# pingooio/pingoo

Measured on AMD Instinct MI355X. Metric: requests/sec matched (whole node), 1k-rule WAF, higher is better.
Workload: dtype u8

## Files before the change

pingoo_amd/build.py:

```python
from __future__ import annotations

import os
import shutil
import subprocess
import sys

HERE = os.path.dirname(os.path.abspath(__file__))
CSRC = os.path.join(HERE, "csrc")
LIB = os.path.join(HERE, "libpwaf.so")
SOURCES = ["frontend.cpp", "pattern.cpp", "dfa.cpp", "iptrie.cpp", "filter.cpp", "residual.cpp", "residual_jit.cpp", "rtc.cpp", "compile.cpp", "loaders.cpp", "batcher.cpp", "async.cpp", "node.cpp", "engine.cpp", "kernels.hip", "records.hip"]
HEADERS = ["frontend.h", "program.h", "kernels.h", "residual.h", "confirm.h", "records.h", "lscan_split.h", "unicode_data.inc", os.path.join("..", "..", "include", "pwaf.h")]


def hipcc() -> str:
    for cand in (os.environ.get("HIPCC"), shutil.which("hipcc"), "/opt/rocm/bin/hipcc"):
        if cand and os.path.exists(cand):
            return cand
    raise RuntimeError("hipcc not found (needed to build pingoo_amd/libpwaf.so)")


EMBED = os.path.join(CSRC, "residual_h.inc")


def embed() -> str:
    text = open(os.path.join(CSRC, "residual.h")).read()
    assert ')RVMH"' not in text
    out = 'R"RVMH(' + text + ')RVMH"\n'
    if not os.path.exists(EMBED) or open(EMBED).read() != out:
        with open(EMBED, "w") as f:
            f.write(out)
    return EMBED


def is_stale(lib: str = LIB) -> bool:
    if not os.path.exists(lib):
        return True
    t = os.path.getmtime(lib)
    return any(os.path.getmtime(os.path.join(CSRC, f)) > t for f in SOURCES + HEADERS)


def build(force: bool = False, verbose: bool = False, variant: str = "") -> str:
    lib = LIB if not variant else os.path.join(HERE, f"libpwaf_{variant}.so")
    if not force and not is_stale(lib):
        return lib
# ... 40 lines not shown
```

pingoo_amd/csrc/engine.cpp:

```cpp
#include <hip/hip_runtime_api.h>

#include <cstdio>
#include <algorithm>
#include <cstring>
#include <functional>
#include <map>
#include <memory>
#include <mutex>
#include <string>
#include <unordered_map>
#include <vector>

#include "frontend.h"
#include "kernels.h"
#include "lscan_split.h"
#include "program.h"
#include "records.h"

using namespace pwaf;

struct pwaf_program {
    std::unique_ptr<Program> p;
    std::vector<uint8_t> dump;
};
// ... 1227 lines not shown
                la[phase].push_back(a);
            }
            if (d.confirm && !d.confirm_walk) continue;
#ifdef PWAF_PROFILING
            if (skip_identity_walks() && d.identity) continue;
#endif
            ListScanArgs a = list_args(gi, lshapes[phase]);
            if (phase == 0 && d.confirm && dense_flag_of[gi] != nullptr) {
                a.dense_flag = dense_flag_of[gi];
                a.dense_thresh = dense_thresh_of[gi];
                a.dense_mode = 2;
            } else if (d.share_owner >= 0 && dense_flag_of[(size_t)d.share_owner] != nullptr) {
                a.dense_flag = dense_flag_of[(size_t)d.share_owner];
                a.dense_thresh = dense_thresh_of[(size_t)d.share_owner];
                a.dense_mode = 3;
            }
            la[phase].push_back(a);
        }
    for (int phase = 0; phase < 2; phase++) {
        size_t planned = 0;
        for (const uint32_t c : e->lscan_launches[phase]) planned += c;
        if (planned != la[phase].size()) return fail(PWAF_E_DEVICE, "list-scan launch plan does not match the batch's descriptors");
    }
    ColPtrChunk ptrs{};
    if (P.n_residual) {
        const size_t nc = e->n_fields;
        ptrs.count = (uint32_t)(2 * nc);
        for (size_t f = 0; f < nc; f++) { ptrs.p[f] = cols[f].data; ptrs.p[nc + f] = cols[f].offsets; }
    }
    const uint32_t nf = (uint32_t)fall.size(), nc_conf = (uint32_t)call.size();
    const FilterArgs *d_all = nullptr, *d_s1 = nullptr, *d_s2 = nullptr;
    const ConfirmArgs *d_c = nullptr;
    const ListScanArgs *d_la[2] = {nullptr, nullptr};
    uint32_t *c_plan = nullptr, *l_plan = nullptr;
    {
        size_t ab = 0;
        auto part = [&](size_t bytes) { const size_t at = ab; ab = (ab + bytes + 255) & ~(size_t)255; return at; };
        const size_t a_all = part((size_t)nf * sizeof(FilterArgs)), a_s1 = part(by_stride[0].size() * sizeof(FilterArgs)), a_s2 = part(by_stride[1].size() * sizeof(FilterArgs)),
                     a_c = part((size_t)nc_conf * sizeof(ConfirmArgs)), a_l0 = part((la[0].size() + 1) * sizeof(ListScanArgs)), a_l1 = part((la[1].size() + 1) * sizeof(ListScanArgs)),
                     a_ptrs = part((size_t)ptrs.count * sizeof(void *));
        const size_t up_bytes = ab;
        const size_t a_cplan = part(((size_t)nc_conf + 2) * 4), a_lplan = part((lsplit::plan_words(e->lscan_launches[0]) + lsplit::plan_words(e->lscan_launches[1])) * 4);
        if ((rc = S.args.reserve(ab))) return rc;
        char *const abase = (char *)S.args.p;
        d_all = (const FilterArgs *)(abase + a_all);
        d_s1 = (const FilterArgs *)(abase + a_s1);
        d_s2 = (const FilterArgs *)(abase + a_s2);
        d_c = (const ConfirmArgs *)(abase + a_c);
        d_la[0] = (const ListScanArgs *)(abase + a_l0);
        d_la[1] = (const ListScanArgs *)(abase + a_l1);
        S.res_cols.p = abase + a_ptrs;
        c_plan = (uint32_t *)(abase + a_cplan);
        l_plan = (uint32_t *)(abase + a_lplan);
        if (up_bytes) {
            const uint32_t slot = S.arg_next++ % Scratch::kArgSlots;
            if (S.arg_pending[slot]) HIP_TRY(hipEventSynchronize(S.arg_ev[slot]));
            if ((rc = S.arg_slot[slot].reserve(up_bytes))) return rc;
            char *const hb = (char *)S.arg_slot[slot].p;
            auto put = [&](size_t at, const void *src, size_t bytes) { if (bytes) memcpy(hb + at, src, bytes); };
            put(a_all, fall.data(), (size_t)nf * sizeof(FilterArgs));
            put(a_s1, by_stride[0].data(), by_stride[0].size() * sizeof(FilterArgs));
            put(a_s2, by_stride[1].data(), by_stride[1].size() * sizeof(FilterArgs));
            put(a_c, call.data(), (size_t)nc_conf * sizeof(ConfirmArgs));
            put(a_l0, la[0].data(), la[0].size() * sizeof(ListScanArgs));
            put(a_l1, la[1].data(), la[1].size() * sizeof(ListScanArgs));
            put(a_ptrs, ptrs.p, (size_t)ptrs.count * sizeof(void *));
            int he = upload_args_block(hb, S.args.p, up_bytes, zero_deferred ? S.zero_block.p : nullptr, zero_deferred ? zero_bytes : 0, stream);
            if (he) return fail(PWAF_E_DEVICE, std::string("descriptor upload failed: ") + hipGetErrorString((hipError_t)he));
            zero_deferred = false;
            arg_slot_used = (int)slot;
        }
        if (zero_deferred) {
            HIP_TRY(hipMemsetAsync(S.zero_block.p, 0, zero_bytes, stream));
            zero_deferred = false;
        }
    }
    if (e->n_filtered) {
        int he;
        stream_mark = true;
        if ((rc = mark(nullptr, 0))) return rc;
        he = launch_filter(by_stride[0].data(), (uint32_t)by_stride[0].size(), d_s1, by_stride[1].data(), (uint32_t)by_stride[1].size(), d_s2, stream);
        if (he) return fail(PWAF_E_DEVICE, std::string("filter kernel launch failed: ") + hipGetErrorString((hipError_t)he));
        if ((rc = mark(by_stride[1].empty() ? "filter_s1" : by_stride[0].empty() ? "filter_s2" : "filter_mix", alg_bytes[1] + alg_bytes[2]))) return rc;
        stream_mark = false;
#ifdef PWAF_PROFILING
        static const bool attr_after_compact = getenv("PWAF_ATTR_AFTER_COMPACT") != nullptr;
        if (!attr_after_compact)
#endif
        if ((rc = launch_attr_side())) return rc;
        if ((rc = mark(nullptr, 0))) return rc;
        he = launch_resolve(fall.data(), nf, d_all, stream);
        bool any_list = false;
        for (const DevGroup &d : e->groups) any_list = any_list || (d.filtered && !d.confirm);
        if (!he && any_list) he = launch_compact(fall.data(), nf, d_all, stream);
        if (he) return fail(PWAF_E_DEVICE, std::string("resolve / compact kernel launch failed: ") + hipGetErrorString((hipError_t)he));
        if ((rc = mark("resolve+compact", 0xFCu))) return rc;
        if (!call.empty()) {
            if ((rc = mark(nullptr, 0))) return rc;
            he = launch_confirm(call.data(), nc_conf, d_c, c_plan, e->n_cus, stream);
            if (he) return fail(PWAF_E_DEVICE, std::string("confirm kernel launch failed: ") + hipGetErrorString((hipError_t)he));
            if ((rc = mark("confirm", 0xF8u))) return rc;
        }
    }
    if ((rc = launch_attr_side())) return rc;
    {
        uint32_t *plan_at = l_plan;
        for (int phase = 0; phase < 2; phase++) {
            uint32_t first = 0;
            for (const uint32_t cnt : e->lscan_launches[phase]) {
                if ((rc = mark(nullptr, 0))) return rc;
                int he = launch_scan_gated(la[phase].data() + first, cnt, d_la[phase] + first, plan_at, lshapes[phase], stream);
                plan_at += 2 * cnt + 1;
                first += cnt;
                if (he) return fail(PWAF_E_DEVICE, std::string("gated scan kernel launch failed: ") + hipGetErrorString((hipError_t)he));
                char nm[48];
                snprintf(nm, sizeof nm, "lscan_x%u", cnt);
                if ((rc = mark(nm, 0xFDu))) return rc;
            }
        }
    }
    if (!P.fcmp.empty()) {
        FcmpArgs fa{};
        std::vector<uint32_t> slots;
        for (size_t k = 0; k < P.fcmp.size(); k++) {
            uint32_t sl[2];
            const uint32_t fld[2] = {P.fcmp[k].a, P.fcmp[k].b};
            for (int q = 0; q < 2; q++) {
                size_t at = std::find(slots.begin(), slots.end(), fld[q]) - slots.begin();
                if (at == slots.size()) slots.push_back(fld[q]);
                sl[q] = (uint32_t)at;
            }
            fa.atoms[k] = P.fcmp[k].op | (sl[0] << 8) | (sl[1] << 16);
        }
        for (size_t q = 0; q < slots.size() && q < kMaxFcmpFields; q++) {
            fa.data[q] = cols[slots[q]].data;
            fa.off[q] = cols[slots[q]].offsets;
        }
        fa.n = n;
        fa.n_atoms = (uint32_t)P.fcmp.size();
        fa.rec = (uint32_t *)S.rec.p + e->groups.size() * (size_t)n;
        fa.pool = (PoolEntry *)S.pool.p;
        fa.pool_count = (uint32_t *)S.ctrl.p;
        fa.pool_cap = pool_cap;
        fa.status = status_word;
        if ((rc = mark(nullptr, 0))) return rc;
// ... 1466 lines not shown
```

pingoo_amd/csrc/kernels.h:

```cpp
#pragma once
#include <cstdint>
#include <string>
#include <vector>

#include "program.h"

namespace pwaf {

static constexpr int kMaxPasses = 250;
static constexpr int kVerdictPre = 12;
static constexpr uint32_t kGapLists = 32;
static constexpr uint32_t kMaxHeaderLens = 8;
static constexpr uint32_t kDirChunkWords = 32;

static constexpr uint32_t REC_OVERFLOW = 0x80000000u;
struct PoolEntry {
    uint32_t atom;
    uint32_t next;
};

struct SpecialCell {
    uint32_t next_off;
    uint32_t emit;
};
// ... 83 lines not shown
    uint32_t pair_cap;
    uint32_t mul, stride, init;
    const uint32_t *ftable;
    const uint32_t *c_head;
    const ConfirmEntry *c_entries;
    const uint8_t *c_bytes;
    const uint32_t *c_classes;
    uint32_t n_entries, n_bytes, n_class_words;
    uint32_t *rec;
    uint32_t *valid_bits;
    uint32_t *walk_bits;
    uint32_t *walk_list;
    uint32_t *walk_count;
    PoolEntry *pool;
    uint32_t *pool_count;
    uint32_t pool_cap;
    uint32_t *status;
    const uint32_t *colmask_local;
    uint32_t n_local;
    uint32_t *gate_lists;
    uint32_t *gate_count;
    uint32_t *enq_bits;
    uint32_t enq_words;
    uint32_t shared_bits;
    const uint32_t *dense_flag;
    uint32_t dense_thresh;
};
static constexpr uint32_t kConfirmThreads = 1024;
static constexpr uint32_t kConfirmPoolBytes = 40 * 1024;
struct ConfirmTableDev {
    const ConfirmArgs *c;
    uint32_t count;
};
int launch_confirm(const ConfirmArgs *host, uint32_t count, const ConfirmArgs *dev, uint32_t *plan, uint32_t n_cus, void *stream);

static constexpr uint32_t kStreamSlab = 128 * 1024;
static constexpr uint32_t kStreamIter = 4096;
static constexpr uint32_t kFilterWaves = 4;
static constexpr uint32_t kCompactWords = 2048;
struct FilterArgs {
    const uint8_t *data;
    const uint32_t *off;
    uint32_t n;
    uint32_t total;
    uint32_t slab0;
    uint32_t init;
    uint32_t mul;
    uint32_t stride;
    const uint32_t *table;
    uint32_t n_heads;
    uint32_t head_w[2][4];
    uint32_t head_m[2][4];
    uint32_t head_len[2];
    uint32_t head_code[2];
    uint32_t *rec;
    uint32_t *chunk_bits;
    uint32_t *sub_count;
    uint32_t *bitmap;
    uint32_t *block_count;
    uint32_t *list;
    uint32_t *list_count;
    uint2 *pairs;
    uint32_t *pair_count;
    uint32_t pair_cap;
    uint32_t *pair_base;
    const uint32_t *dense_flag;
    uint32_t dense_thresh;
// ... 147 lines not shown
    const uint32_t *dir24;
    const uint32_t *dir_chunks, *dir_vals;
    const uint32_t *dir_summary;
    uint32_t dir_sum_shift, dir_common;
    const uint2 *dir_esc;
    const uint32_t *class_rows;
    uint32_t class_words;
    uint32_t acmp_words;
    uint32_t geo_default;
    uint32_t *ipres;
    uint32_t ipres_packed;
    uint32_t has_geo;
    uint4 *gpairs;
    uint32_t *ghdr;
    uint32_t pair_stride;
    uint32_t attr_blocks;
    pwaf_verdict *out;
    unsigned long long *counts;
    uint32_t *match_idx;
    uint32_t *n_matches;
};

int launch_scan(const ScanArgs &a, void *stream);
struct GatedTable {
    const ListScanArgs *g;
    uint32_t count;
    uint32_t debug;
};
struct ListShape {
    uint32_t threads, hot_bytes, wg_per_cu;
};
ListShape list_shape(uint32_t variant);
uint32_t list_hot_bytes(const ListShape &shape);
int launch_scan_gated(const ListScanArgs *host, uint32_t count, const ListScanArgs *dev, uint32_t *plan, const ListShape &shape, void *stream);
int launch_verdict(const VerdictArgs &a, void *stream);
int launch_ipres(const VerdictArgs &a, void *stream);
int launch_attr(const VerdictArgs &a, void *stream);
int launch_dir24(const VerdictArgs &a, void *out , void *esc, void *esc_count, void *stream);
uint32_t scan_lds_bytes(uint32_t n_hot, uint32_t stride, uint32_t n_gate_atoms);
struct VerdictShape {
    uint32_t waves, lds_bytes, lds_tables;
    uint32_t sparse, v_cap, per_cu;
};
VerdictShape verdict_shape(uint32_t n_cols, uint32_t n_rules, uint32_t n_trig, uint32_t n_lits, bool force_global = false, int mode = 3, uint32_t n_passes = 0);
uint32_t verdict_blocks_sp(const VerdictShape &sh, uint32_t n_cus);

}
```

pingoo_amd/csrc/kernels.hip:

```cpp
#include <hip/hip_runtime.h>

#include <cstdlib>
#include <mutex>
#include <set>

#include "confirm.h"
#include "utf8.h"
#include "kernels.h"
#include "residual.h"

namespace pwaf {

static constexpr int kScanThreads = 1024;
static constexpr int kScanWaves = kScanThreads / 64;
static constexpr uint32_t kNone = 0xFFFFFFFFu;

#define PWAF_LDS __attribute__((address_space(3)))
#define PWAF_GLOBAL __attribute__((address_space(1)))
typedef const PWAF_LDS uint16_t *lds_u16_ptr;
typedef const PWAF_GLOBAL uint16_t *glb_u16_ptr;
typedef const PWAF_LDS uint32_t *lds_u32_ptr;
typedef const PWAF_LDS uint8_t *lds_u8_ptr;
typedef unsigned int u32x4 __attribute__((ext_vector_type(4)));
typedef u32x4 u32x4_u __attribute__((aligned(1)));

static constexpr uint32_t kClsBytes = 1024;
uint32_t scan_lds_bytes(uint32_t n_hot, uint32_t stride, uint32_t n_gate_atoms) {
    const uint32_t need = (((n_hot + 1) * stride * 2 + 15) & ~15u) + kClsBytes + n_gate_atoms * 4;
    const uint32_t reach = ((0xFFFFu << 1) + stride * 2 + kClsBytes + 15) & ~15u;
    return need > reach ? need : reach;
}


struct Hits {
    uint32_t a0, a1;
    uint32_t ovf;
};

struct SlowCtx {
    const uint32_t *list_off;
    const uint16_t *list;
    PoolEntry *pool;
// ... 354 lines not shown
            r = kNone;
        }
        if (r == kNone && r2 != kNone) {
            r = r2;
            p = p2;
            end = end2;
            r2 = kNone;
            row = 0;
            h = Hits{0, 0, kNone};
            if (start_emit) PWAF_EMIT(start_emit - 1);
        }
#pragma unroll
        for (int q = 0; q < CH; q++) w[q] = wn[q];
        n_lo = f_lo;
        n_hi = f_hi;
        n_base = f_base;
    }
}

template <int CH, bool WIDE>
__global__ __launch_bounds__(kScanThreads) void scan_kernel(ScanArgs a) { scan_body<CH, WIDE>(a); }

__device__ __forceinline__ ListOf list_of(const ListScanArgs &a) {
    ListOf l{a.req_list, a.req_list != nullptr ? min(*a.n_list, a.n) : a.n};
    if (a.dense_mode != 0u) {
        const bool dense = *a.dense_flag > a.dense_thresh;
        if (a.dense_mode == 1u && !dense) l.n_l = 0u;
        if (a.dense_mode == 2u && dense) l.n_l = 0u;
        if (a.dense_mode == 3u && dense) l = ListOf{nullptr, a.n};
    }
    return l;
}

__global__ __launch_bounds__(256) void lscan_plan_kernel(GatedTable b, uint32_t *plan , uint32_t n_waves) {
    __shared__ uint32_t part[256];
    __shared__ unsigned long long all_entries;
    const uint32_t t = threadIdx.x;
    uint32_t items = 0;
    const uint32_t n_l = t < b.count ? list_of(b.g[t]).n_l : 0u;
    if (t == 0) all_entries = 0ull;
    __syncthreads();
    if (n_l != 0u) atomicAdd(&all_entries, (unsigned long long)n_l);
    __syncthreads();
    if (t < b.count) {
        const uint32_t room = n_waves > b.count ? n_waves - b.count : 1u;
        const unsigned long long per_wave = (all_entries + room - 1u) / room;
        uint32_t epi = 1;
        while (epi < 16u && epi < per_wave) epi <<= 1;
        while (epi < 64u * kListWalks && (n_l + epi - 1) / epi > n_waves) epi <<= 1;
        items = (n_l + epi - 1) / epi;
        plan[b.count + 1 + t] = epi;
    }
    part[t] = items;
    __syncthreads();
    for (uint32_t d = 1; d < 256; d <<= 1) {
        const uint32_t v = t >= d ? part[t - d] : 0u;
        __syncthreads();
        part[t] += v;
        __syncthreads();
    }
    if (t < b.count) plan[t] = part[t] - items;
    if (t == 0) plan[b.count] = part[255];
}

__device__ __forceinline__ uint32_t list_step_slow(const uint16_t *hot, const PWAF_GLOBAL uint16_t *flat, const uint64_t *delta, const uint32_t state, const uint32_t c,
                                                   const uint32_t stride, const uint32_t n_hot, const uint32_t n_delta) {
    if (state < n_hot) return hot[state * stride + c];
    const uint32_t k = state - n_hot;
    if (k < n_delta) {
        if (c + 2u == stride) return state;
        const uint64_t rec = delta[k];
        const uint32_t lo = (uint32_t)rec, hi = (uint32_t)(rec >> 32);
        if (c == ((lo >> 16) & 0xFFu)) return hi & 0xFFFFu;
        if (c == (lo >> 24)) return hi >> 16;
        return hot[(lo & 0xFFFFu) * stride + c];
    }
    return flat[state * stride + c];
}

template <uint32_t THREADS>
__device__ __forceinline__ void lscan_async(const ListScanArgs &a, const uint16_t *hot, const unsigned char *cls, const uint64_t *delta, uint32_t it, const uint32_t it_end,
                                            const uint32_t first, const uint32_t n_l, const uint32_t hot_elems, const uint32_t epi) {
    const uint32_t ncls = a.n_classes, stride = ncls + 3u;
    const PWAF_GLOBAL unsigned char *gdata = (const PWAF_GLOBAL unsigned char *)a.data;
    const PWAF_GLOBAL uint16_t *flat = (const PWAF_GLOBAL uint16_t *)a.flat;
    auto record_emit = [&](const uint32_t st, Hits &hh) {
        const uint32_t ei = st * stride + ncls;
        const uint32_t code = ei < hot_elems ? (uint32_t)hot[ei] : (uint32_t)flat[ei];
        const uint32_t x = (code & 0x7FFFu) + 1u;
        bool slow = !(code & 0x8000u) || hh.ovf != kNone;
        if (!slow) {
            if (hh.a0 == x || hh.a1 == x) {}
            else if (hh.a0 == 0) hh.a0 = x;
            else if (hh.a1 == 0) hh.a1 = x;
            else slow = true;
// ... 59 lines not shown
                    if (any & 0x8000u) {
#pragma unroll
                        for (uint32_t k = 0; k < 4; k++)
                            if (t[k] & 0x8000u) record_emit(sv[k], h);
                    }
                    state = sv[3];
                    p += 4u;
                }
            } else if (blocked) {
#pragma unroll
                for (uint32_t k = 0; k < 4; k++) {
                    const uint32_t tt = list_step_slow(hot, flat, delta, state, c[k], stride, a.n_hot, a.n_delta);
                    state = tt & 0x7FFFu;
                    if (tt & 0x8000u) record_emit(state, h);
                }
                p += 4u;
            }
        }
        if (live) {
            if (a.end_off[state + 1] != a.end_off[state]) h = emit_list(a.end_off, a.end_list, a.pool, a.pool_count, a.status, a.pool_cap, state, h);
            a.rec[r] = h.ovf != kNone ? (REC_OVERFLOW | h.ovf) : (h.a0 | (h.a1 << 15));
            if (a.colmask_local != nullptr) {
                uint32_t need = 0;
                if ((h.a0 | (h.ovf + 1u)) != 0) need = gate_mask(a.colmask_local, a.pool, h);
                if (a.need_out != nullptr) a.need_out[li] = need;
                need &= ~(a.shared_bits | need_init);
                if (need) enqueue_mask_once(a.gate_lists, a.gate_count, a.n, r, need, a.enq_bits, a.enq_words);
            }
        }
    }
}

template <uint32_t THREADS>
__global__ __launch_bounds__(THREADS, THREADS == 512 ? 6 : 4) void lscan_kernel(GatedTable b, const uint32_t *plan, uint32_t hot_bytes) {
    extern __shared__ uint32_t lscan_lds[];
    __builtin_amdgcn_s_setprio(3);
    if ((uint32_t)(uintptr_t)(PWAF_LDS unsigned char *)lscan_lds != 0u) __builtin_trap();
    const uint32_t total = plan[b.count];
    const uint32_t it0 = (uint32_t)((uint64_t)total * blockIdx.x / gridDim.x), it1 = (uint32_t)((uint64_t)total * (blockIdx.x + 1) / gridDim.x);
    const unsigned char *cls = reinterpret_cast<const unsigned char *>(lscan_lds + (hot_bytes + 16u) / 4);
    const uint16_t *hot = reinterpret_cast<const uint16_t *>(lscan_lds);
    for (uint32_t it = it0; it < it1;) {
        uint32_t ps = 0;
        for (uint32_t lo = 0, hi = b.count; lo + 1 < hi;) {
            const uint32_t mid = (lo + hi) >> 1;
            if (plan[mid] <= it) lo = mid;
            else hi = mid;
            ps = lo;
        }
        const uint32_t first = plan[ps], it_end = min(it1, plan[ps + 1]), epi = plan[b.count + 1 + ps];
        ListScanArgs a = load_descriptor(&b.g[ps]);
        const ListOf lst = list_of(a);
        a.req_list = lst.req_list;
        const uint32_t ncls = a.n_classes, stride = ncls + 3u;
        const uint32_t hot_elems = a.n_hot * stride;
        uint64_t *delta_lds = reinterpret_cast<uint64_t *>(lscan_lds) + (hot_elems * 2u + 2u + 15u) / 16u * 2u;
        __syncthreads();
        {
            const uint4 *src = reinterpret_cast<const uint4 *>(a.flat);
            uint4 *dst = reinterpret_cast<uint4 *>(lscan_lds);
            const uint32_t units = (hot_elems * 2u + 15u) / 16u;
            for (uint32_t k = threadIdx.x; k < units; k += THREADS * 4u) {
                uint4 v[4];
#pragma unroll
                for (uint32_t q = 0; q < 4; q++) v[q] = k + q * THREADS < units ? src[k + q * THREADS] : make_uint4(0u, 0u, 0u, 0u);
#pragma unroll
                for (uint32_t q = 0; q < 4; q++)
                    if (k + q * THREADS < units) dst[k + q * THREADS] = v[q];
            }
            if (threadIdx.x < 64) lscan_lds[(hot_bytes + 16u) / 4 + threadIdx.x] = reinterpret_cast<const uint32_t *>(a.classmap)[threadIdx.x];
            for (uint32_t k = threadIdx.x; k < a.n_delta; k += THREADS) delta_lds[k] = a.delta[k];
        }
        __syncthreads();
        if (threadIdx.x == 0) reinterpret_cast<uint16_t *>(lscan_lds)[hot_elems] = 0xFFFFu;
        __syncthreads();
        const uint32_t n_l = lst.n_l;
#ifdef PWAF_PROFILING
        const bool long_list = (b.debug & 1u) ? false : (b.debug & 2u) ? true : (a.behind_filter != 0u && (uint64_t)n_l * 8u >= a.n);
#else
        const bool long_list = a.behind_filter != 0u && (uint64_t)n_l * 8u >= a.n;
#endif
        if (long_list) {
            lscan_async<THREADS>(a, hot, cls, delta_lds, it, it_end, first, n_l, hot_elems, epi);
// ... 111 lines not shown
#pragma unroll
                                for (uint32_t k = 0; k < 4; k++)
                                    if (t[u][k] & 0x8000u) record_emit(sv[u][k], h[u]);
                                state[u] = sv[u][3];
                            }
                        }
                    } else {
#pragma unroll
                        for (uint32_t u = 0; u < kListWalks; u++) state[u] = sv[u][3];
                    }
                }
#pragma unroll
                for (uint32_t u = 0; u < kListWalks; u++) {
                    if (p[u] < end[u]) p[u] += 16u;
                    w[u] = wn[u];
                }
            }
#pragma unroll
            for (uint32_t u = 0; u < kListWalks; u++) {
                if (!live[u]) continue;
                if (a.end_off[state[u] + 1] != a.end_off[state[u]]) h[u] = emit_list(a.end_off, a.end_list, a.pool, a.pool_count, a.status, a.pool_cap, state[u], h[u]);
                a.rec[r[u]] = h[u].ovf != kNone ? (REC_OVERFLOW | h[u].ovf) : (h[u].a0 | (h[u].a1 << 15));
                if (a.colmask_local != nullptr) {
                    uint32_t need = 0;
                    if ((h[u].a0 | (h[u].ovf + 1u)) != 0) need = gate_mask(a.colmask_local, a.pool, h[u]);
                    if (a.need_out != nullptr) a.need_out[li[u]] = need;
                    need &= ~(a.shared_bits | need_init[u]);
                    if (need) enqueue_mask_once(a.gate_lists, a.gate_count, a.n, r[u], need, a.enq_bits, a.enq_words);
                }
            }
        }
        it = it_end;
    }
}

__global__ __launch_bounds__(256) void confirm_plan_kernel(ConfirmTableDev b, uint32_t *plan ) {
    __shared__ uint32_t part[256];
    const uint32_t t = threadIdx.x;
    uint32_t items = 0;
    if (t < b.count) {
        const ConfirmArgs *pa = &b.c[t];
        const bool dense = pa->dense_flag != nullptr && *pa->dense_flag > pa->dense_thresh;
        items = dense ? 0u : (min(*pa->pair_count, pa->pair_cap) + kConfirmThreads - 1) / kConfirmThreads;
    }
    part[t] = items;
    __syncthreads();
    for (uint32_t d = 1; d < 256; d <<= 1) {
        const uint32_t v = t >= d ? part[t - d] : 0u;
        __syncthreads();
        part[t] += v;
        __syncthreads();
    }
    if (t < b.count) plan[t] = part[t] - items;
    if (t == 0) plan[b.count] = part[255];
}

__device__ __noinline__ void merge_atom(PoolEntry *pool, uint32_t *pool_count, uint32_t *status, uint32_t pool_cap, uint32_t *rec, uint32_t atom) {
    auto rmw_read = [](uint32_t *p) { return atomicOr(p, 0u); };
    auto publish = [&](uint32_t idx, uint32_t at, uint32_t next) {
        const uint32_t t0 = atomicExch(&pool[idx].atom, at), t1 = atomicExch(&pool[idx].next, next);
        asm volatile("" ::"v"(t0), "v"(t1));
    };
    uint32_t old = rmw_read(rec);
    for (;;) {
        uint32_t upd;
        const uint32_t x = atom + 1u;
        if (!(old & REC_OVERFLOW)) {
            const uint32_t a0 = old & 0x7FFFu, a1 = (old >> 15) & 0x7FFFu;
            if (a0 == x || a1 == x) return;
            if (a0 == 0u) upd = old | x;
            else if (a1 == 0u) upd = old | (x << 15);
            else {
                const uint32_t idx = atomicAdd(pool_count, 3u);
                if (idx + 3u > pool_cap) { atomicOr(status, 1u); return; }
                publish(idx, a0 - 1u, kNone);
                publish(idx + 1u, a1 - 1u, idx);
                publish(idx + 2u, atom, idx + 1u);
                upd = REC_OVERFLOW | (idx + 2u);
            }
        } else {
            const uint32_t head = old & ~REC_OVERFLOW;
            for (uint32_t i = head; i != kNone; i = rmw_read(&pool[i].next))
                if (rmw_read(&pool[i].atom) == atom) return;
            const uint32_t idx = atomicAdd(pool_count, 1u);
            if (idx >= pool_cap) { atomicOr(status, 1u); return; }
            publish(idx, atom, head);
            upd = REC_OVERFLOW | idx;
        }
        const uint32_t seen = atomicCAS(rec, old, upd);
        if (seen == old) return;
        old = seen;
    }
}

__global__ __launch_bounds__(kConfirmThreads, 8) void confirm_kernel(ConfirmTableDev b, const uint32_t *plan) {
    __shared__ uint32_t head[kFilterEntries], ftab[kFilterEntries];
    __shared__ uint32_t pool[kConfirmPoolBytes / 4];
    constexpr uint32_t kConfirmQueue = 1024;
    __shared__ uint32_t app_cnt, app_base, app_queue[kConfirmQueue];
    __builtin_amdgcn_s_setprio(3);
    if (threadIdx.x == 0) app_cnt = 0;
    const uint32_t total = plan[b.count];
    const uint32_t it0 = (uint32_t)((uint64_t)total * blockIdx.x / gridDim.x), it1 = (uint32_t)((uint64_t)total * (blockIdx.x + 1) / gridDim.x);
    for (uint32_t it = it0; it < it1;) {
        uint32_t ps = 0;
        for (uint32_t lo = 0, hi = b.count; lo + 1 < hi;) {
            const uint32_t mid = (lo + hi) >> 1;
            if (plan[mid] <= it) lo = mid;
            else hi = mid;
            ps = lo;
        }
        const uint32_t first_item = plan[ps], it_end = min(it1, plan[ps + 1]);
        const ConfirmArgs a = load_descriptor(&b.c[ps]);
        __syncthreads();
        {
            const uint4 *sh = reinterpret_cast<const uint4 *>(a.c_head), *sf = reinterpret_cast<const uint4 *>(a.ftable);
            constexpr uint32_t kPer = kFilterEntries / 4 / kConfirmThreads;
            uint4 vh[kPer], vf[kPer];
#pragma unroll
            for (uint32_t q = 0; q < kPer; q++) { vh[q] = sh[q * kConfirmThreads + threadIdx.x]; vf[q] = sf[q * kConfirmThreads + threadIdx.x]; }
#pragma unroll
            for (uint32_t q = 0; q < kPer; q++) {
                reinterpret_cast<uint4 *>(head)[q * kConfirmThreads + threadIdx.x] = vh[q];
                reinterpret_cast<uint4 *>(ftab)[q * kConfirmThreads + threadIdx.x] = vf[q];
            }
        }
        const uint32_t e_words = a.n_entries * 3u, b_words = a.n_bytes / 4u, c_words = a.n_class_words;
        const bool in_lds = (uint64_t)e_words + b_words + c_words <= kConfirmPoolBytes / 4;
        const ConfirmEntry *t_entries = a.c_entries;
        const uint8_t *t_bytes = a.c_bytes;
        const uint32_t *t_classes = a.c_classes;
        if (in_lds) {
            const uint32_t *se = reinterpret_cast<const uint32_t *>(a.c_entries), *sb = reinterpret_cast<const uint32_t *>(a.c_bytes);
            for (uint32_t k = threadIdx.x; k < e_words; k += kConfirmThreads) pool[k] = se[k];
            for (uint32_t k = threadIdx.x; k < b_words; k += kConfirmThreads) pool[e_words + k] = sb[k];
            for (uint32_t k = threadIdx.x; k < c_words; k += kConfirmThreads) pool[e_words + b_words + k] = a.c_classes[k];
            t_entries = reinterpret_cast<const ConfirmEntry *>(pool);
            t_bytes = reinterpret_cast<const uint8_t *>(pool + e_words);
            t_classes = pool + e_words + b_words;
        }
        __syncthreads();
        const ConfirmView cv{nullptr, t_entries, t_bytes, t_classes, a.mul, a.stride, a.init};
        const uint32_t n_p = min(*a.pair_count, a.pair_cap);
        auto pair_of = [&](const uint32_t item) -> uint2 {
            const uint32_t k = (item - first_item) * kConfirmThreads + threadIdx.x;
// ... 96 lines not shown
    const int v = (a.chunks == 4 ? 2 : a.chunks == 2 ? 1 : 0) + (wide ? 3 : 0);
    const void *fns[6] = {reinterpret_cast<const void *>(scan_kernel<1, false>), reinterpret_cast<const void *>(scan_kernel<2, false>),
                          reinterpret_cast<const void *>(scan_kernel<4, false>), reinterpret_cast<const void *>(scan_kernel<1, true>),
                          reinterpret_cast<const void *>(scan_kernel<2, true>), reinterpret_cast<const void *>(scan_kernel<4, true>)};
    const void *fn = fns[v];
    if (a.n == 0) return 0;
    uint32_t waves = (a.n + 255) / 256;
    uint32_t blocks = (waves + kScanWaves - 1) / kScanWaves;
#ifdef PWAF_PROFILING
    static const uint32_t forced_cap = getenv("PWAF_SCAN_BLOCKS") ? (uint32_t)atoi(getenv("PWAF_SCAN_BLOCKS")) : 0u;
#else
    const uint32_t forced_cap = 0;
#endif
    const uint32_t cap = forced_cap ? forced_cap : std::max(1u, a.n_cus);
    if (blocks > cap) blocks = cap;
    if (blocks == 0) blocks = 1;
    void *args[] = {const_cast<ScanArgs *>(&a)};
    hipError_t e = hipLaunchKernel(fn, dim3(blocks), dim3(kScanThreads), args, lds, (hipStream_t)stream);
    return (int)(e != hipSuccess ? e : hipGetLastError());
}

__global__ __launch_bounds__(256) void copy_args_kernel(const uint4 *__restrict__ src, uint4 *__restrict__ dst, uint32_t n16, uint4 *__restrict__ zero, uint32_t z16) {
    for (uint32_t i = blockIdx.x * 256u + threadIdx.x; i < n16; i += gridDim.x * 256u) dst[i] = src[i];
    for (uint32_t i = blockIdx.x * 256u + threadIdx.x; i < z16; i += gridDim.x * 256u) zero[i] = make_uint4(0u, 0u, 0u, 0u);
}
int upload_args_block(const void *host_pinned, void *dev, size_t bytes, void *zero, size_t zero_bytes, void *stream) {
    const uint32_t n16 = (uint32_t)((bytes + 15) / 16), z16 = (uint32_t)(zero_bytes / 16);
    if (n16 == 0 && z16 == 0) return 0;
    const uint32_t blocks = std::max(std::min<uint32_t>((n16 + 255) / 256, 64u), std::min<uint32_t>((z16 + 2047) / 2048, 1024u));
    hipLaunchKernelGGL(copy_args_kernel, dim3(std::max(1u, blocks)), dim3(256), 0, (hipStream_t)stream, (const uint4 *)host_pinned, (uint4 *)dev, n16, (uint4 *)zero, z16);
    return (int)hipGetLastError();
}

int launch_confirm(const ConfirmArgs *host, uint32_t count, const ConfirmArgs *dev, uint32_t *plan, uint32_t n_cus, void *stream) {
    if (count == 0 || host[0].n == 0) return 0;
    if (count > 256) return (int)hipErrorInvalidValue;
    ConfirmTableDev b{dev, count};
    hipLaunchKernelGGL(confirm_plan_kernel, dim3(1), dim3(256), 0, (hipStream_t)stream, b, plan);
    hipError_t e = hipGetLastError();
    if (e != hipSuccess) return (int)e;
    uint64_t max_items = 0;
    for (uint32_t k = 0; k < count; k++) max_items += ((uint64_t)host[k].pair_cap + kConfirmThreads - 1) / kConfirmThreads;
    const uint32_t blocks = (uint32_t)std::min<uint64_t>(max_items, (uint64_t)std::max(1u, n_cus) * 2u);
    const uint32_t *cplan = plan;
    hipLaunchKernelGGL(confirm_kernel, dim3(blocks), dim3(kConfirmThreads), 0, (hipStream_t)stream, b, cplan);
    return (int)hipGetLastError();
}

static const void *lscan_fn(bool wide) { return wide ? reinterpret_cast<const void *>(lscan_kernel<1024>) : reinterpret_cast<const void *>(lscan_kernel<512>); }

int launch_scan_gated(const ListScanArgs *host, uint32_t count, const ListScanArgs *dev, uint32_t *plan, const ListShape &shape, void *stream) {
    if (count == 0 || host[0].n == 0) return 0;
    if (count > 256) return (int)hipErrorInvalidValue;
    GatedTable b{dev, count, 0u};
#ifdef PWAF_PROFILING
    static const uint32_t async_mode = getenv("PWAF_LSCAN_ASYNC") ? (uint32_t)atoi(getenv("PWAF_LSCAN_ASYNC")) : 0u;
    b.debug = async_mode;
#endif
    const uint32_t blocks = std::max(1u, host[0].n_cus) * shape.wg_per_cu;
    hipLaunchKernelGGL(lscan_plan_kernel, dim3(1), dim3(256), 0, (hipStream_t)stream, b, plan, blocks * (shape.threads / 64u));
    hipError_t e = hipGetLastError();
    if (e != hipSuccess) return (int)e;
    const uint32_t *cplan = plan;
    uint32_t hot_bytes = list_hot_bytes(shape);
    void *args[] = {&b, &cplan, &hot_bytes};
    const void *fn = lscan_fn(shape.threads == 1024);
    e = hipLaunchKernel(fn, dim3(blocks), dim3(shape.threads), args, shape.hot_bytes + 16 + 256, (hipStream_t)stream);
    return (int)(e != hipSuccess ? e : hipGetLastError());
}

uint32_t list_hot_bytes(const ListShape &shape) { return shape.hot_bytes; }

ListShape list_shape(uint32_t variant) {
    switch (variant) {
        case 1: return ListShape{512, 72u * 1024u, 2};
        case 2: return ListShape{1024, 144u * 1024u, 1};
        case 3: return ListShape{512, 32u * 1024u, 4};
        default: return ListShape{kListThreads, kListHotBytes, 3};
    }
}

typedef unsigned short u16x2 __attribute__((ext_vector_type(2)));

template <bool HEADS, int STRIDE>
__device__ __forceinline__ void filter_rows(const FilterArgs &a, const uint32_t blk, const uint32_t wave, const uint32_t lane) {
    const PWAF_GLOBAL unsigned char *gdata = (const PWAF_GLOBAL unsigned char *)a.data;
    const uint32_t rel = blk * kFilterWaves + wave, slab = a.slab0 + rel;
    const uint64_t base64 = (uint64_t)slab * kStreamSlab;
    if (base64 >= a.total) return;
    const uint32_t total = a.total, base0 = (uint32_t)base64, slab_end = (uint32_t)min<uint64_t>(total, base64 + kStreamSlab);
    unsigned long long *my_bits = reinterpret_cast<unsigned long long *>(a.chunk_bits) + (size_t)rel * (kStreamSlab / 1024);
    uint32_t n_hit = 0;
    const uint32_t mul2 = a.mul | (a.mul << 16);
    constexpr uint32_t kRow = 1024;

    auto load_row = [&](const uint32_t b, const uint32_t q) {
        const uint32_t p = b + kRow * q + 16u * lane;
        return *reinterpret_cast<const PWAF_GLOBAL u32x4_u *>(gdata + (p < total ? p : 0u));
    };
    auto dword_at = [&](const uint32_t p) {
// ... 2160 lines not shown
```

Before: 7.132 billion.

## Fold confirm and list-scan planning kernels into the main kernels via per-block LDS scans

Drops the separate single-block plan kernels for the confirm and list-scan stages. Each block of the main kernel now recomputes the prefix-sum work plan in shared memory with a wave-level scan, and the plan lookups are made uniform with readfirstlane. This removes two kernel launches per stage, along with their device plan buffers and the serialization between plan and work kernels. The cost is redundant plan computation in every block, extra LDS for the list-scan kernel that may lower occupancy, and extra barriers at kernel start.

```diff
diff --git a/pingoo_amd/build.py b/pingoo_amd/build.py
--- a/pingoo_amd/build.py
+++ b/pingoo_amd/build.py
@@ -9,7 +9,7 @@
 CSRC = os.path.join(HERE, "csrc")
 LIB = os.path.join(HERE, "libpwaf.so")
 SOURCES = ["frontend.cpp", "pattern.cpp", "dfa.cpp", "iptrie.cpp", "filter.cpp", "residual.cpp", "residual_jit.cpp", "rtc.cpp", "compile.cpp", "loaders.cpp", "batcher.cpp", "async.cpp", "node.cpp", "engine.cpp", "kernels.hip", "records.hip"]
-HEADERS = ["frontend.h", "program.h", "kernels.h", "residual.h", "confirm.h", "records.h", "lscan_split.h", "unicode_data.inc", os.path.join("..", "..", "include", "pwaf.h")]
+HEADERS = ["frontend.h", "program.h", "kernels.h", "residual.h", "confirm.h", "records.h", "lscan_split.h", "work_plan.h", "unicode_data.inc", os.path.join("..", "..", "include", "pwaf.h")]
 
 
 def hipcc() -> str:
diff --git a/pingoo_amd/csrc/engine.cpp b/pingoo_amd/csrc/engine.cpp
--- a/pingoo_amd/csrc/engine.cpp
+++ b/pingoo_amd/csrc/engine.cpp
@@ -1283,7 +1283,6 @@
     const FilterArgs *d_all = nullptr, *d_s1 = nullptr, *d_s2 = nullptr;
     const ConfirmArgs *d_c = nullptr;
     const ListScanArgs *d_la[2] = {nullptr, nullptr};
-    uint32_t *c_plan = nullptr, *l_plan = nullptr;
     {
         size_t ab = 0;
         auto part = [&](size_t bytes) { const size_t at = ab; ab = (ab + bytes + 255) & ~(size_t)255; return at; };
@@ -1291,7 +1290,6 @@
                      a_c = part((size_t)nc_conf * sizeof(ConfirmArgs)), a_l0 = part((la[0].size() + 1) * sizeof(ListScanArgs)), a_l1 = part((la[1].size() + 1) * sizeof(ListScanArgs)),
                      a_ptrs = part((size_t)ptrs.count * sizeof(void *));
         const size_t up_bytes = ab;
-        const size_t a_cplan = part(((size_t)nc_conf + 2) * 4), a_lplan = part((lsplit::plan_words(e->lscan_launches[0]) + lsplit::plan_words(e->lscan_launches[1])) * 4);
         if ((rc = S.args.reserve(ab))) return rc;
         char *const abase = (char *)S.args.p;
         d_all = (const FilterArgs *)(abase + a_all);
@@ -1301,8 +1299,6 @@
         d_la[0] = (const ListScanArgs *)(abase + a_l0);
         d_la[1] = (const ListScanArgs *)(abase + a_l1);
         S.res_cols.p = abase + a_ptrs;
-        c_plan = (uint32_t *)(abase + a_cplan);
-        l_plan = (uint32_t *)(abase + a_lplan);
         if (up_bytes) {
             const uint32_t slot = S.arg_next++ % Scratch::kArgSlots;
             if (S.arg_pending[slot]) HIP_TRY(hipEventSynchronize(S.arg_ev[slot]));
@@ -1348,20 +1344,18 @@
         if ((rc = mark("resolve+compact", 0xFCu))) return rc;
         if (!call.empty()) {
             if ((rc = mark(nullptr, 0))) return rc;
-            he = launch_confirm(call.data(), nc_conf, d_c, c_plan, e->n_cus, stream);
+            he = launch_confirm(call.data(), nc_conf, d_c, e->n_cus, stream);
             if (he) return fail(PWAF_E_DEVICE, std::string("confirm kernel launch failed: ") + hipGetErrorString((hipError_t)he));
             if ((rc = mark("confirm", 0xF8u))) return rc;
         }
     }
     if ((rc = launch_attr_side())) return rc;
     {
-        uint32_t *plan_at = l_plan;
         for (int phase = 0; phase < 2; phase++) {
             uint32_t first = 0;
             for (const uint32_t cnt : e->lscan_launches[phase]) {
                 if ((rc = mark(nullptr, 0))) return rc;
-                int he = launch_scan_gated(la[phase].data() + first, cnt, d_la[phase] + first, plan_at, lshapes[phase], stream);
-                plan_at += 2 * cnt + 1;
+                int he = launch_scan_gated(la[phase].data() + first, cnt, d_la[phase] + first, lshapes[phase], stream);
                 first += cnt;
                 if (he) return fail(PWAF_E_DEVICE, std::string("gated scan kernel launch failed: ") + hipGetErrorString((hipError_t)he));
                 char nm[48];
diff --git a/pingoo_amd/csrc/kernels.h b/pingoo_amd/csrc/kernels.h
--- a/pingoo_amd/csrc/kernels.h
+++ b/pingoo_amd/csrc/kernels.h
@@ -139,7 +139,7 @@
     const ConfirmArgs *c;
     uint32_t count;
 };
-int launch_confirm(const ConfirmArgs *host, uint32_t count, const ConfirmArgs *dev, uint32_t *plan, uint32_t n_cus, void *stream);
+int launch_confirm(const ConfirmArgs *host, uint32_t count, const ConfirmArgs *dev, uint32_t n_cus, void *stream);
 
 static constexpr uint32_t kStreamSlab = 128 * 1024;
 static constexpr uint32_t kStreamIter = 4096;
@@ -353,7 +353,7 @@
 };
 ListShape list_shape(uint32_t variant);
 uint32_t list_hot_bytes(const ListShape &shape);
-int launch_scan_gated(const ListScanArgs *host, uint32_t count, const ListScanArgs *dev, uint32_t *plan, const ListShape &shape, void *stream);
+int launch_scan_gated(const ListScanArgs *host, uint32_t count, const ListScanArgs *dev, const ListShape &shape, void *stream);
 int launch_verdict(const VerdictArgs &a, void *stream);
 int launch_ipres(const VerdictArgs &a, void *stream);
 int launch_attr(const VerdictArgs &a, void *stream);
diff --git a/pingoo_amd/csrc/kernels.hip b/pingoo_amd/csrc/kernels.hip
--- a/pingoo_amd/csrc/kernels.hip
+++ b/pingoo_amd/csrc/kernels.hip
@@ -8,6 +8,7 @@
 #include "utf8.h"
 #include "kernels.h"
 #include "residual.h"
+#include "work_plan.h"
 
 namespace pwaf {
 
@@ -428,35 +429,42 @@
     return l;
 }
 
-__global__ __launch_bounds__(256) void lscan_plan_kernel(GatedTable b, uint32_t *plan , uint32_t n_waves) {
-    __shared__ uint32_t part[256];
-    __shared__ unsigned long long all_entries;
+__device__ __forceinline__ uint32_t wave_scan_add(uint32_t x);
+
+__device__ __forceinline__ void plan_scan(const uint32_t items, const uint32_t count, uint32_t *first, uint32_t *wave_tot) {
     const uint32_t t = threadIdx.x;
+    uint32_t incl = 0;
+    if (t < wplan::kPlanMax) {
+        incl = wave_scan_add(items);
+        if ((t & 63u) == 63u) wave_tot[t >> 6] = incl;
+    }
+    __syncthreads();
+    if (t < wplan::kPlanMax) {
+        uint32_t before = 0;
+        for (uint32_t w = 0; w < (t >> 6); w++) before += wave_tot[w];
+        if (t < count) first[t] = before + incl - items;
+        if (t == wplan::kPlanMax - 1u) first[count] = before + incl;
+    }
+    __syncthreads();
+}
+
+static constexpr uint32_t kListPlanBytes = (8u + 4u * (wplan::kPlanMax / 64u) + 4u * wplan::kPlanWords + 15u) / 16u * 16u;
+__device__ __forceinline__ void lscan_plan(const GatedTable &b, uint32_t *area, const uint32_t n_waves) {
+    unsigned long long *all_entries = reinterpret_cast<unsigned long long *>(area);
+    uint32_t *wave_tot = area + 2, *plan = wave_tot + wplan::kPlanMax / 64u;
+    const uint32_t t = threadIdx.x;
+    const uint32_t n_l = t < b.count ? list_of(b.g[t]).n_l : 0u;
+    if (t == 0) *all_entries = 0ull;
+    __syncthreads();
+    if (n_l != 0u) atomicAdd(all_entries, (unsigned long long)n_l);
+    __syncthreads();
     uint32_t items = 0;
-    const uint32_t n_l = t < b.count ? list_of(b.g[t]).n_l : 0u;
-    if (t == 0) all_entries = 0ull;
-    __syncthreads();
-    if (n_l != 0u) atomicAdd(&all_entries, (unsigned long long)n_l);
-    __syncthreads();
     if (t < b.count) {
-        const uint32_t room = n_waves > b.count ? n_waves - b.count : 1u;
-        const unsigned long long per_wave = (all_entries + room - 1u) / room;
-        uint32_t epi = 1;
-        while (epi < 16u && epi < per_wave) epi <<= 1;
-        while (epi < 64u * kListWalks && (n_l + epi - 1) / epi > n_waves) epi <<= 1;
-        items = (n_l + epi - 1) / epi;
+        const uint32_t epi = wplan::list_epi(n_l, wplan::list_epi_floor(*all_entries, n_waves, b.count), n_waves, 64u * kListWalks);
+        items = wplan::list_items(n_l, epi);
         plan[b.count + 1 + t] = epi;
     }
-    part[t] = items;
-    __syncthreads();
-    for (uint32_t d = 1; d < 256; d <<= 1) {
-        const uint32_t v = t >= d ? part[t - d] : 0u;
-        __syncthreads();
-        part[t] += v;
-        __syncthreads();
-    }
-    if (t < b.count) plan[t] = part[t] - items;
-    if (t == 0) plan[b.count] = part[255];
+    plan_scan(items, b.count, plan, wave_tot);
 }
 
 __device__ __forceinline__ uint32_t list_step_slow(const uint16_t *hot, const PWAF_GLOBAL uint16_t *flat, const uint64_t *delta, const uint32_t state, const uint32_t c,
@@ -582,23 +590,21 @@
 }
 
 template <uint32_t THREADS>
-__global__ __launch_bounds__(THREADS, THREADS == 512 ? 6 : 4) void lscan_kernel(GatedTable b, const uint32_t *plan, uint32_t hot_bytes) {
+__global__ __launch_bounds__(THREADS, THREADS == 512 ? 6 : 4) void lscan_kernel(GatedTable b, uint32_t hot_bytes) {
     extern __shared__ uint32_t lscan_lds[];
     __builtin_amdgcn_s_setprio(3);
     if ((uint32_t)(uintptr_t)(PWAF_LDS unsigned char *)lscan_lds != 0u) __builtin_trap();
-    const uint32_t total = plan[b.count];
+    uint32_t *const plan_area = lscan_lds + (hot_bytes + 16u + 256u) / 4;
+    lscan_plan(b, plan_area, gridDim.x * (THREADS / 64u));
+    const uint32_t *plan = plan_area + 2 + wplan::kPlanMax / 64u;
+    auto uni = [](const uint32_t x) { return (uint32_t)__builtin_amdgcn_readfirstlane((int)x); };
+    const uint32_t total = uni(plan[b.count]);
     const uint32_t it0 = (uint32_t)((uint64_t)total * blockIdx.x / gridDim.x), it1 = (uint32_t)((uint64_t)total * (blockIdx.x + 1) / gridDim.x);
     const unsigned char *cls = reinterpret_cast<const unsigned char *>(lscan_lds + (hot_bytes + 16u) / 4);
     const uint16_t *hot = reinterpret_cast<const uint16_t *>(lscan_lds);
     for (uint32_t it = it0; it < it1;) {
-        uint32_t ps = 0;
-        for (uint32_t lo = 0, hi = b.count; lo + 1 < hi;) {
-            const uint32_t mid = (lo + hi) >> 1;
-            if (plan[mid] <= it) lo = mid;
-            else hi = mid;
-            ps = lo;
-        }
-        const uint32_t first = plan[ps], it_end = min(it1, plan[ps + 1]), epi = plan[b.count + 1 + ps];
+        const uint32_t ps = uni(wplan::pass_of_item(plan, b.count, it));
+        const uint32_t first = uni(plan[ps]), it_end = min(it1, uni(plan[ps + 1])), epi = uni(plan[b.count + 1 + ps]);
         ListScanArgs a = load_descriptor(&b.g[ps]);
         const ListOf lst = list_of(a);
         a.req_list = lst.req_list;
@@ -776,27 +782,6 @@
         }
         it = it_end;
     }
-}
-
-__global__ __launch_bounds__(256) void confirm_plan_kernel(ConfirmTableDev b, uint32_t *plan ) {
-    __shared__ uint32_t part[256];
-    const uint32_t t = threadIdx.x;
-    uint32_t items = 0;
-    if (t < b.count) {
-        const ConfirmArgs *pa = &b.c[t];
-        const bool dense = pa->dense_flag != nullptr && *pa->dense_flag > pa->dense_thresh;
-        items = dense ? 0u : (min(*pa->pair_count, pa->pair_cap) + kConfirmThreads - 1) / kConfirmThreads;
-    }
-    part[t] = items;
-    __syncthreads();
-    for (uint32_t d = 1; d < 256; d <<= 1) {
-        const uint32_t v = t >= d ? part[t - d] : 0u;
-        __syncthreads();
-        part[t] += v;
-        __syncthreads();
-    }
-    if (t < b.count) plan[t] = part[t] - items;
-    if (t == 0) plan[b.count] = part[255];
 }
 
 __device__ __noinline__ void merge_atom(PoolEntry *pool, uint32_t *pool_count, uint32_t *status, uint32_t pool_cap, uint32_t *rec, uint32_t atom) {
@@ -837,24 +822,29 @@
     }
 }
 
-__global__ __launch_bounds__(kConfirmThreads, 8) void confirm_kernel(ConfirmTableDev b, const uint32_t *plan) {
+__global__ __launch_bounds__(kConfirmThreads, 8) void confirm_kernel(ConfirmTableDev b) {
     __shared__ uint32_t head[kFilterEntries], ftab[kFilterEntries];
     __shared__ uint32_t pool[kConfirmPoolBytes / 4];
     constexpr uint32_t kConfirmQueue = 1024;
     __shared__ uint32_t app_cnt, app_base, app_queue[kConfirmQueue];
+    __shared__ uint32_t plan[wplan::kPlanMax + 1], plan_wave[wplan::kPlanMax / 64];
     __builtin_amdgcn_s_setprio(3);
     if (threadIdx.x == 0) app_cnt = 0;
-    const uint32_t total = plan[b.count];
+    {
+        uint32_t items = 0;
+        if (threadIdx.x < b.count) {
+            const ConfirmArgs *pa = &b.c[threadIdx.x];
+            const bool dense = pa->dense_flag != nullptr && *pa->dense_flag > pa->dense_thresh;
+            items = wplan::confirm_items(dense ? 0u : *pa->pair_count, pa->pair_cap, dense, kConfirmThreads);
+        }
+        plan_scan(items, b.count, plan, plan_wave);
+    }
+    auto uni = [](const uint32_t x) { return (uint32_t)__builtin_amdgcn_readfirstlane((int)x); };
+    const uint32_t total = uni(plan[b.count]);
     const uint32_t it0 = (uint32_t)((uint64_t)total * blockIdx.x / gridDim.x), it1 = (uint32_t)((uint64_t)total * (blockIdx.x + 1) / gridDim.x);
     for (uint32_t it = it0; it < it1;) {
-        uint32_t ps = 0;
-        for (uint32_t lo = 0, hi = b.count; lo + 1 < hi;) {
-            const uint32_t mid = (lo + hi) >> 1;
-            if (plan[mid] <= it) lo = mid;
-            else hi = mid;
-            ps = lo;
-        }
-        const uint32_t first_item = plan[ps], it_end = min(it1, plan[ps + 1]);
+        const uint32_t ps = uni(wplan::pass_of_item(plan, b.count, it));
+        const uint32_t first_item = uni(plan[ps]), it_end = min(it1, uni(plan[ps + 1]));
         const ConfirmArgs a = load_descriptor(&b.c[ps]);
         __syncthreads();
         {
@@ -1017,40 +1007,32 @@
     return (int)hipGetLastError();
 }
 
-int launch_confirm(const ConfirmArgs *host, uint32_t count, const ConfirmArgs *dev, uint32_t *plan, uint32_t n_cus, void *stream) {
+int launch_confirm(const ConfirmArgs *host, uint32_t count, const ConfirmArgs *dev, uint32_t n_cus, void *stream) {
     if (count == 0 || host[0].n == 0) return 0;
-    if (count > 256) return (int)hipErrorInvalidValue;
+    if (count > wplan::kPlanMax) return (int)hipErrorInvalidValue;
     ConfirmTableDev b{dev, count};
-    hipLaunchKernelGGL(confirm_plan_kernel, dim3(1), dim3(256), 0, (hipStream_t)stream, b, plan);
-    hipError_t e = hipGetLastError();
-    if (e != hipSuccess) return (int)e;
     uint64_t max_items = 0;
     for (uint32_t k = 0; k < count; k++) max_items += ((uint64_t)host[k].pair_cap + kConfirmThreads - 1) / kConfirmThreads;
     const uint32_t blocks = (uint32_t)std::min<uint64_t>(max_items, (uint64_t)std::max(1u, n_cus) * 2u);
-    const uint32_t *cplan = plan;
-    hipLaunchKernelGGL(confirm_kernel, dim3(blocks), dim3(kConfirmThreads), 0, (hipStream_t)stream, b, cplan);
+    hipLaunchKernelGGL(confirm_kernel, dim3(blocks), dim3(kConfirmThreads), 0, (hipStream_t)stream, b);
     return (int)hipGetLastError();
 }
 
 static const void *lscan_fn(bool wide) { return wide ? reinterpret_cast<const void *>(lscan_kernel<1024>) : reinterpret_cast<const void *>(lscan_kernel<512>); }
 
-int launch_scan_gated(const ListScanArgs *host, uint32_t count, const ListScanArgs *dev, uint32_t *plan, const ListShape &shape, void *stream) {
+int launch_scan_gated(const ListScanArgs *host, uint32_t count, const ListScanArgs *dev, const ListShape &shape, void *stream) {
     if (count == 0 || host[0].n == 0) return 0;
-    if (count > 256) return (int)hipErrorInvalidValue;
+    if (count > wplan::kPlanMax) return (int)hipErrorInvalidValue;
     GatedTable b{dev, count, 0u};
 #ifdef PWAF_PROFILING
     static const uint32_t async_mode = getenv("PWAF_LSCAN_ASYNC") ? (uint32_t)atoi(getenv("PWAF_LSCAN_ASYNC")) : 0u;
     b.debug = async_mode;
 #endif
     const uint32_t blocks = std::max(1u, host[0].n_cus) * shape.wg_per_cu;
-    hipLaunchKernelGGL(lscan_plan_kernel, dim3(1), dim3(256), 0, (hipStream_t)stream, b, plan, blocks * (shape.threads / 64u));
-    hipError_t e = hipGetLastError();
-    if (e != hipSuccess) return (int)e;
-    const uint32_t *cplan = plan;
     uint32_t hot_bytes = list_hot_bytes(shape);
-    void *args[] = {&b, &cplan, &hot_bytes};
+    void *args[] = {&b, &hot_bytes};
     const void *fn = lscan_fn(shape.threads == 1024);
-    e = hipLaunchKernel(fn, dim3(blocks), dim3(shape.threads), args, shape.hot_bytes + 16 + 256, (hipStream_t)stream);
+    hipError_t e = hipLaunchKernel(fn, dim3(blocks), dim3(shape.threads), args, shape.hot_bytes + 16 + 256 + kListPlanBytes, (hipStream_t)stream);
     return (int)(e != hipSuccess ? e : hipGetLastError());
 }
 
diff --git a/pingoo_amd/csrc/work_plan.h b/pingoo_amd/csrc/work_plan.h
--- /dev/null
+++ b/pingoo_amd/csrc/work_plan.h
@@ -0,0 +1,71 @@
+#pragma once
+#include <stddef.h>
+#include <stdint.h>
+
+#if defined(__HIPCC__)
+#define PWAF_PLAN_HD __host__ __device__ __forceinline__
+#else
+#define PWAF_PLAN_HD inline
+#endif
+
+namespace pwaf {
+namespace wplan {
+
+static constexpr uint32_t kPlanMax = 256;
+static constexpr uint32_t kEpiFloorMax = 16;
+static constexpr uint32_t kPlanWords = 2 * kPlanMax + 1;
+
+PWAF_PLAN_HD uint32_t confirm_items(uint32_t pair_count, uint32_t pair_cap, bool dense, uint32_t threads) {
+    if (dense) return 0u;
+    const uint32_t pairs = pair_count < pair_cap ? pair_count : pair_cap;
+    return pairs / threads + (pairs % threads != 0u ? 1u : 0u);
+}
+
+PWAF_PLAN_HD uint32_t list_items(uint32_t n_l, uint32_t epi) { return n_l / epi + (n_l % epi != 0u ? 1u : 0u); }
+PWAF_PLAN_HD uint32_t list_epi_floor(uint64_t all_entries, uint32_t n_waves, uint32_t count) {
+    const uint32_t room = n_waves > count ? n_waves - count : 1u;
+    const uint64_t per_wave = (all_entries + room - 1u) / room;
+    uint32_t epi = 1;
+    while (epi < kEpiFloorMax && epi < per_wave) epi <<= 1;
+    return epi;
+}
+PWAF_PLAN_HD uint32_t list_epi(uint32_t n_l, uint32_t floor_epi, uint32_t n_waves, uint32_t max_epi) {
+    uint32_t epi = floor_epi;
+    while (epi < max_epi && list_items(n_l, epi) > n_waves) epi <<= 1;
+    return epi;
+}
+
+PWAF_PLAN_HD uint32_t pass_of_item(const uint32_t *first, uint32_t count, uint32_t it) {
+    uint32_t ps = 0;
+    for (uint32_t lo = 0, hi = count; lo + 1 < hi;) {
+        const uint32_t mid = (lo + hi) >> 1;
+        if (first[mid] <= it) lo = mid;
+        else hi = mid;
+        ps = lo;
+    }
+    return ps;
+}
+
+inline void confirm_plan(const uint32_t *pair_count, const uint32_t *pair_cap, const uint8_t *dense, uint32_t count, uint32_t threads, uint32_t *first ) {
+    uint32_t acc = 0;
+    for (uint32_t t = 0; t < count; t++) {
+        first[t] = acc;
+        acc += confirm_items(pair_count[t], pair_cap[t], dense[t] != 0, threads);
+    }
+    first[count] = acc;
+}
+inline void list_plan(const uint32_t *n_l, uint32_t count, uint32_t n_waves, uint32_t max_epi, uint32_t *first , uint32_t *epi ) {
+    uint64_t all_entries = 0;
+    for (uint32_t t = 0; t < count; t++) all_entries += n_l[t];
+    const uint32_t floor_epi = list_epi_floor(all_entries, n_waves, count);
+    uint32_t acc = 0;
+    for (uint32_t t = 0; t < count; t++) {
+        epi[t] = list_epi(n_l[t], floor_epi, n_waves, max_epi);
+        first[t] = acc;
+        acc += list_items(n_l[t], epi[t]);
+    }
+    first[count] = acc;
+}
+
+}
+}
```

Result: no change. 7.123 billion (-0.1%).
